# niess/turtle

Hardware: AMD Instinct MI355X
Metric: ray-steps/sec (whole node) through 3601^2 SRTM tile (higher is better)
Workload: dtype f64

## Files before the change

### turtle_amd/csrc/device.hip

```cpp
#include <hip/hip_runtime.h>
#include <hipcub/device/device_radix_sort.hpp>

#include <cfloat>
#include <cstdio>
#include <cstdlib>
#include <cstring>
#include <type_traits>

#include "device_ctx.h"
#include "internal.h"
#include "trace_room.h"

using namespace turtle_amd_device;

namespace {


__device__ __forceinline__ int lane_rank(ull mask)
{
        return __builtin_amdgcn_mbcnt_hi((unsigned)(mask >> 32), __builtin_amdgcn_mbcnt_lo((unsigned)mask, 0));
}

struct RayQueue {
        long next = 0, end = 0;
// ... 2157 lines not shown
        }
        block_tally(stats, my_rays, my_steps, my_samples, my_capped);
}

__global__ void k_traverse_gen(long n, int first, const double * __restrict__ alt,
    const double * __restrict__ step, int * __restrict__ live_index, int * __restrict__ medium,
    int * __restrict__ index, double * __restrict__ length, int * __restrict__ n_steps,
    int * __restrict__ n_cross, double ceiling, int max_steps, ull * __restrict__ counters)
{
        ull my_rays = 0, my_steps = 0, my_capped = 0, my_live = 0;
        for (long r = blockIdx.x * (long)blockDim.x + threadIdx.x; r < n;
             r += (long)gridDim.x * blockDim.x) {
                const int m1 = live_index[2 * r];
                int count = 0;
                if (first) {
                        n_steps[r] = 0, n_cross[r] = 0;
                } else {
                        const int m0 = medium[r];
                        if (m0 < 0) continue;
                        if (length != nullptr) length[(long)m0 * n + r] += step[r];
                        count = n_steps[r] + 1;
                        n_steps[r] = count;
                        n_cross[r] += (m1 != m0) ? 1 : 0;
                        my_steps++;
                }
                index[2 * r] = m1, index[2 * r + 1] = live_index[2 * r + 1];
                const bool low = (m1 >= 0) && (alt[r] < ceiling);
                if (!low || (count >= max_steps)) {
                        medium[r] = -1, live_index[2 * r] = -1;
                        my_rays++;
                        my_capped += low ? 1 : 0;
                } else {
                        medium[r] = m1;
                        my_live++;
                }
        }
        block_tally(counters, my_rays, my_steps, my_capped, my_live);
}

__global__ void k_crossings_gen(long n, const double * __restrict__ pos, const double * __restrict__ step,
    const int * __restrict__ live_index, const int * __restrict__ medium, const int * __restrict__ n_cross,
    double * __restrict__ total, tamd_crossings rec)
{
        for (long r = blockIdx.x * (long)blockDim.x + threadIdx.x; r < n;
             r += (long)gridDim.x * blockDim.x) {
                const int m0 = medium[r];
                if (m0 < 0) continue;
                const double tot = total[r] + step[r];
                total[r] = tot;
                const int m1 = live_index[2 * r];
                if ((m1 != m0) && (n_cross[r] < rec.capacity)) {
                        const long c = (long)n_cross[r] * n + r;
                        if (rec.point != nullptr)
                                rec.point[3 * c] = pos[3 * r], rec.point[3 * c + 1] = pos[3 * r + 1],
                                rec.point[3 * c + 2] = pos[3 * r + 2];
                        if (rec.distance != nullptr) rec.distance[c] = tot;
                        if (rec.media != nullptr) rec.media[2 * c] = m0, rec.media[2 * c + 1] = m1;
                }
        }
}

__global__ void k_philox(long n, ull seed, ull stream, long first, unsigned * __restrict__ out)
{
        for (long r = blockIdx.x * (long)blockDim.x + threadIdx.x; r < n;
             r += (long)gridDim.x * blockDim.x) {
                const ull id = (ull)(first + r);
                unsigned c[4] = { (unsigned)id, (unsigned)(id >> 32), (unsigned)stream,
                        (unsigned)(stream >> 32) };
                philox4x32_10(c, (unsigned)seed, (unsigned)(seed >> 32));
                for (int i = 0; i < 4; i++) out[4 * r + i] = c[i];
        }
}

__global__ void k_isotropic(long n, ull seed, ull stream, long first, double * __restrict__ dir)
{
        for (long r = blockIdx.x * (long)blockDim.x + threadIdx.x; r < n;
             r += (long)gridDim.x * blockDim.x) {
                double x, y, z;
                d_isotropic((ull)(first + r), stream, seed, x, y, z);
                dir[3 * r] = x, dir[3 * r + 1] = y, dir[3 * r + 2] = z;
        }
}

__global__ void __launch_bounds__(256) k_tally(long n, const int * __restrict__ index,
    const double * __restrict__ length, int n_media, ull * __restrict__ hits,
    int n_bins, double scale, ull * __restrict__ histogram)
{
        extern __shared__ unsigned int lds[];
        unsigned int * h_hits = lds;
        unsigned int * h_bins = lds + (n_media + 1);
        const int total = n_media + 1 + n_bins + 1;
        for (int i = threadIdx.x; i < total; i += blockDim.x) lds[i] = 0;
        __syncthreads();
        for (long r = blockIdx.x * (long)blockDim.x + threadIdx.x; r < n;
             r += (long)gridDim.x * blockDim.x) {
                const int m = index[2 * r];
                if ((m >= -1) && (m < n_media)) atomicAdd(&h_hits[m + 1], 1u);
                const double t = length[r] * scale;
                int b = n_bins;
                if ((t >= 0.) && (t < (double)n_bins)) b = (int)t;
                atomicAdd(&h_bins[b], 1u);
        }
        __syncthreads();
        for (int i = threadIdx.x; i < total; i += blockDim.x) {
                const unsigned int c = lds[i];
                if (c == 0) continue;
                if (i <= n_media)
                        atomicAdd(&hits[i], (ull)c);
                else
                        atomicAdd(&histogram[i - (n_media + 1)], (ull)c);
        }
}

enum { RS_STACK = 0, RS_MAP = 1 };

__device__ __forceinline__ void page_fault_block(const Paging & pg, const TileFault & f, int item)
{
        const bool fault = f.centre >= 0;
        const ull mask = __ballot(fault);
        if (mask == 0) return;
        const int lane = (int)(threadIdx.x & 63);
        const int leader = __builtin_ctzll(mask);
        ull base = 0;
        if (lane == leader) {
                base = atomicAdd(pg.n_faulted, 1ull);
                pg.faulted[base] = item;
        }
        base = __shfl(base, leader, 64);
        const bool first = (pg.first_id >= 0) ? (item == pg.first_id) : (base == 0);
        if (fault) {
                for (int b = 0; b < 9; b++) {
                        if (!((f.mask >> b) & 1)) continue;
                        const int t = f.centre + (b / 3 - 1) * f.stride + (b % 3 - 1);
                        if (b != 4) atomicAdd(&pg.wanted[(size_t)t * TAMD_DEMAND_STRIDE], 1u);
                        if (first) atomicOr(&pg.wanted_first[t >> 5], 1u << (t & 31));
                }
        }
        const bool centre = fault && (((f.mask >> 4) & 1) != 0);
        ull left = __ballot(centre);
        while (left != 0) {
                const int lead = __builtin_ctzll(left);
                const int t0 = __shfl(f.centre, lead, 64);
                const ull same = __ballot(centre && (f.centre == t0));
                if (lane == lead) atomicAdd(&pg.wanted[(size_t)t0 * TAMD_DEMAND_STRIDE], 1u);
                left &= ~same;
        }
}

template <int SRC, int TPROJ >
__global__ void __launch_bounds__(256) k_resample(tamd_view v, const tamd_grid * __restrict__ grids,
    double z0, double dz, int is_signed, int flags, long n_blocks, uint16_t * __restrict__ out, Paging pg,
    ull * __restrict__ counters)
{
        const tamd_grid & t = grids[0];
        const int lane = (int)(threadIdx.x & 63);
        const long waves = (long)gridDim.x * (blockDim.x >> 6);
        const long n_items = (pg.n_in != nullptr) ? (long)*pg.n_in : n_blocks;
        const double top = z0 + 65535 * dz;
        ull n_outside = 0, n_bad = 0, n_clamped = 0;
        for (long i = blockIdx.x * (long)(blockDim.x >> 6) + (threadIdx.x >> 6); i < n_items; i += waves) {
                const long blk = (pg.ids != nullptr) ? (long)pg.ids[i] : i;
                const int ix = (int)(blk % t.nbx) * TAMD_BLOCK + (lane & 7);
                const int iy = (int)(blk / t.nbx) * TAMD_BLOCK + (lane >> 3);
                TileFault f = { -1, 0, 0 };
                bool keep = true;
                int outside = 0, bad = 0, clamped = 0;
                uint16_t code = 0;
                if ((ix < t.nx) && (iy < t.ny)) {
                        const double x = t.x0 + ix * t.dx;
                        const double y = t.y0 + iy * t.dy;
                        double latitude, longitude;
                        if (TPROJ >= 0)
                                d_unproject_body<TPROJ>(t.proj, x, y, latitude, longitude);
                        else
                                latitude = y, longitude = x;
                        double z = 0.;
                        int in;
                        if (SRC == RS_STACK) {
                                in = d_stack_elevation<false>(v, v.stacks[0], latitude, longitude, z, f);
                                if (in >= 0) f.centre = -1;
                        } else {
                                const tamd_grid & s = grids[1];
                                double u, w;
                                if (flags & TAMD_RESAMPLE_IDENTITY)
                                        u = x, w = y;
                                else if (s.proj.type >= 0)
                                        d_project_body(s.proj, latitude, longitude, u, w);
                                else
                                        u = longitude, w = latitude;
                                in = d_grid_elevation<false>(s, u, w, z) ? 1 : 0;
                        }
                        if (in == 0) {
                                outside = 1;
                        } else if (in > 0) {
// ... 57 lines not shown
                        if (is_signed)
                                code = (uint16_t)(int)z;
                        else
                                code = (dz > 0.) ? (uint16_t)(unsigned)round((z - z0) / dz) : 0;
                }
                codes[k] = code;
        }
        block_tally(counters, n_bad, n_clamped, n_inconsistent, 0);
}

__global__ void __launch_bounds__(256) k_fill_store(uint16_t * __restrict__ nodes, int nbx, int ix0, int iy0,
    int nx, int ny, int nwx, long n_blocks, int blank, const uint16_t * __restrict__ codes)
{
        const int lane = (int)(threadIdx.x & 63);
        const long waves = (long)gridDim.x * (blockDim.x >> 6);
        for (long i = blockIdx.x * (long)(blockDim.x >> 6) + (threadIdx.x >> 6); i < n_blocks; i += waves) {
                const int bx = (ix0 >> 3) + (int)(i % nwx), by = (iy0 >> 3) + (int)(i / nwx);
                const int ix = bx * TAMD_BLOCK + (lane & 7) - ix0, iy = by * TAMD_BLOCK + (lane >> 3) - iy0;
                const size_t k = ((size_t)by * nbx + bx) * 64 + lane;
                uint16_t code = 0;
                if ((ix >= 0) && (ix < nx) && (iy >= 0) && (iy < ny))
                        code = codes[(long)iy * nx + ix];
                else if (!blank)
                        code = GLOBAL_NODES(nodes)[k];
                nodes[k] = code;
        }
}

__global__ void __launch_bounds__(256) k_nodes(const uint16_t * __restrict__ nodes, int nbx, int ix0, int iy0,
    int nx, long n, double z0, double dz, int is_signed, double * __restrict__ out, long ld)
{
        for (long k = blockIdx.x * (long)blockDim.x + threadIdx.x; k < n; k += (long)gridDim.x * blockDim.x) {
                const long j = k / nx;
                const int i = (int)(k - j * nx);
                const uint16_t code = GLOBAL_NODES(nodes)[d_node_index(nbx, ix0 + i, iy0 + (int)j)];
                out[j * ld + i] = is_signed ? (double)(int16_t)code : z0 + code * dz;
        }
}

}


#define g_stream (g_ctx.stream)
#define g_cus (g_ctx.cus)
#define g_math_strict (g_ctx.math_strict)

#ifdef TRACE_POOL_STATS
extern "C" int tamd_dev_pool_stats(unsigned long long * out, int reset)
{
        HIP_TRY(hipMemcpyFromSymbol(out, HIP_SYMBOL(g_pool_stats), sizeof(g_pool_stats)));
        if (reset) {
                static unsigned long long zero[32];
                HIP_TRY(hipMemcpyToSymbol(HIP_SYMBOL(g_pool_stats), zero, sizeof(zero)));
        }
        return 0;
}
#endif

static int grid_for(long n, int block)
{
        long blocks = (n + block - 1) / block;
        const long cap = (long)(g_cus > 0 ? g_cus : 256) * 8;
        if (blocks > cap) blocks = cap;
        if (blocks < 1) blocks = 1;
        return (int)blocks;
}

template <class... P, class... A>
static int launch_blocks(const char * name, void (*kernel)(P...), unsigned blocks, size_t lds_bytes,
    const A &... args)
{
        hipLaunchKernelGGL(kernel, dim3(blocks), dim3(256), lds_bytes, g_stream, args...);
        LAUNCH_CHECK(name);
        return 0;
}
template <class... P, class... A>
static int launch_items(const char * name, void (*kernel)(P...), long n, size_t lds_bytes, const A &... args)
{
        if (tamd_dev_init()) return 1;
        if (n <= 0) return 0;
        return launch_blocks(name, kernel, grid_for(n, 256), lds_bytes, args...);
}

template <int FIRST, int... REST, class F>
static int with_constant(int value, F && f)
{
        if constexpr (sizeof...(REST) > 0)
                if (value != FIRST) return with_constant<REST...>(value, f);
        return f(std::integral_constant<int, FIRST>());
}
template <class F>
static int with_mode(int mode, F && f)
{
        return with_constant<TAMD_MODE_ONE_MAP, TAMD_MODE_ONE_STACK, TAMD_MODE_GENERIC>(mode, f);
}

typedef std::integral_constant<int, 0> Strict;
typedef std::integral_constant<int, 1> Fast;
template <class F>
static int with_math(bool strict, F && f)
{
        return with_constant<Strict::value, Fast::value>(strict ? Strict::value : Fast::value, f);
}

extern "C" int tamd_k_ecef_from_geodetic(long n, const double * lat,
    const double * lon, const double * elev, double * ecef)
{
        return launch_items("k_ecef_from_geodetic", k_ecef_from_geodetic, n, 0, n, lat, lon, elev, ecef);
}

extern "C" int tamd_k_ecef_to_geodetic(
    long n, const double * ecef, double * lat, double * lon, double * alt)
{
        return with_math(g_math_strict, [&](auto fast) {
                return launch_items("k_ecef_to_geodetic", k_ecef_to_geodetic<decltype(fast)::value>, n, 0, n,
                    ecef, lat, lon, alt);
        });
}

extern "C" int tamd_k_ecef_from_horizontal(long n, const double * lat,
    const double * lon, const double * az, const double * el, double * dir)
{
        return launch_items("k_ecef_from_horizontal", k_ecef_from_horizontal, n, 0, n, lat, lon, az, el, dir);
}

extern "C" int tamd_k_ecef_to_horizontal(long n, const double * lat,
    const double * lon, const double * dir, double * az, double * el)
{
        return launch_items("k_ecef_to_horizontal", k_ecef_to_horizontal, n, 0, n, lat, lon, dir, az, el);
}

extern "C" int tamd_k_elevation(struct tamd_view view, long n, const double * a,
    const double * b, double * z, int * inside, struct tamd_paging pg)
{
        return launch_items("k_elevation", k_elevation, n, 0, view, n, a, b, z, inside, pg);
}

extern "C" int tamd_k_project(struct tamd_proj proj, int inverse, long n, const double * a,
    const double * b, double * c, double * d)
{
        return launch_items("k_project", k_project, n, 0, proj, inverse, n, a, b, c, d);
}

extern "C" int tamd_k_gradient(struct tamd_view view, long n, const double * a,
    const double * b, double * ga, double * gb, int * inside, struct tamd_paging pg)
{
        return launch_items("k_gradient", k_gradient, n, 0, view, n, a, b, ga, gb, inside, pg);
}

extern "C" int tamd_k_position(struct tamd_view view, long n, const double * lat,
    const double * lon, const double * height, int layer, double * pos,
    int * data_index, struct tamd_paging pg)
{
        return launch_items("k_position", k_position, n, 0, view, n, lat, lon, height, layer, pos,
            data_index, pg);
}

extern "C" int tamd_k_normal(struct tamd_view view, long n, const double * pos, const int * layer,
    double * normal, int * data_index, struct tamd_paging pg)
{
        return with_mode(view.mode, [&](auto mode) {
                return launch_items("k_normal", k_normal<decltype(mode)::value>, n, 0, view, n, pos, layer,
                    normal, data_index, pg);
        });
}

// ... 124 lines not shown
        }
        if constexpr (FAST && MODEL && (MODE != TAMD_MODE_GENERIC))
                if (cross && (ph.pool > 0)) return launch_trace_<MODE, FAST, MODEL, false, true, true>(TRACE_ARGS);
        if (cross) return launch_trace_<MODE, FAST, MODEL, false, true>(TRACE_ARGS);
        if constexpr (!MODEL) return launch_trace_<MODE, FAST, MODEL, false, false>(TRACE_ARGS);
        return 1;
#undef TRACE_ARGS
}

struct TraceRays {
        double * pos;
        const double * dir;
        int * index;
        double * length;
        int * n_steps;
};

template <int MODE, bool FAST>
static int launch_cross(struct tamd_view view, long n, const TraceRays & rays, CrossList cross, Paging pg,
    ull * stats, RayOut out = { nullptr, nullptr, nullptr, nullptr, nullptr }, CrossTail front = { nullptr })
{
        constexpr bool CAN_PAGE = (MODE != TAMD_MODE_ONE_MAP);
        const bool paged = CAN_PAGE && (pg.faulted != nullptr);
        const auto kernel = paged ? k_cross<MODE, FAST, CAN_PAGE> : k_cross<MODE, FAST, false>;
        return launch_blocks("k_cross", kernel, persistent_blocks(kernel, n), 0, view, rays.pos, rays.dir, rays.index,
            rays.length, rays.n_steps, cross, pg, stats, out, front, n);
}


struct Knob {
        const char * name;
        long fallback;
        bool read = false;
        long value = 0;
        long get()
        {
                if (!read) {
                        const char * env = getenv(name);
                        value = ((env != nullptr) && (*env != 0)) ? atol(env) : fallback;
                        read = true;
                }
                return value;
        }
};

static int park_threshold(int mode)
{
        static Knob knob = { "TURTLE_AMD_PARK", -1 };
        const int value = (int)knob.get();
        if (value >= 0) return value;
        return (mode == TAMD_MODE_GENERIC) ? 512 : 32;
}
static int creep_lanes(long n)
{
        static Knob knob = { "TURTLE_AMD_CREEP_LANES", -1 };
        const int value = (int)knob.get();
        if (value >= 0) return value;
        return (n >= 2000000) ? 4 * kCreepLanes : kCreepLanes;
}
static int dense_go(void)
{
        static Knob knob = { "TURTLE_AMD_DENSE_GO", 24 };
        return (int)knob.get();
}
static int sort_long_if(void)
{
        static Knob knob = { "TURTLE_AMD_SORT_LONG", 120 };
        return (int)knob.get();
}
static int pool_on(int mode, long n)
{
        static Knob knob = { "TURTLE_AMD_POOL", -1 };
        const int value = (int)knob.get();
        if (value >= 0) return value;
        return (mode == TAMD_MODE_ONE_MAP) && (n >= 6000000);
}
static int sort_hand_over(long n)
{
        static Knob knob = { "TURTLE_AMD_SORT_KEY", -1 };
        const long value = knob.get();
        if (value == 0) return 0;
        if (value == 1) return 1;
        return n <= ((value > 1) ? value : 4000000L);
}
static int spatial_order(int mode, long n)
{
        static Knob knob = { "TURTLE_AMD_SPATIAL", -1 };
        const long value = knob.get();
        if ((mode == TAMD_MODE_GENERIC) || (value == 0)) return 0;
        if (value == 1) return 1;
        return n >= ((value > 1) ? value : 3000000L);
}
static int cross_tail_on(long n)
{
        static Knob knob = { "TURTLE_AMD_CROSS_TAIL", -1 };
        const long value = knob.get();
        if (value >= 0) return value != 0;
        return (g_ctx.in_flight <= 1) && (n <= 3000000L);
}
constexpr int kDrainLanes = 64;
static bool first_pass_flat(int park, bool again, const Paging & pg)
{
        static Knob knob = { "TURTLE_AMD_FIRST_PASS", -1 };
        if (knob.get() == 0) return false;
        return !again && (pg.faulted == nullptr) && (park > 0) && (park <= 64);
}
static int first_pass_waves(bool ordered)
{
        static Knob knob = { "TURTLE_AMD_FIRST_WAVES", -1 };
        if (knob.get() > 0) return (knob.get() <= 3) ? 3 : 8;
        return ordered ? 8 : 3;
}
template <int MODE>
static int launch_first(struct tamd_view view, long n, double * pos, const double * dir, int max_steps,
    int * index, double * length, int * n_steps, int flags, const FirstPass & fp, const RayOut & out, ull * stats)
{
        static Knob grid = { "TURTLE_AMD_FIRST_GRID", 1 };
        if (tamd_dev_init()) return 1;
        const unsigned blocks = (grid.get() == 0) ? (unsigned)grid_for(n, 256) : (unsigned)((n + 255) / 256);
        return with_constant<3, 8>(first_pass_waves(out.order_of != nullptr), [&](auto waves) {
                return launch_blocks("k_first", k_first<MODE, decltype(waves)::value>, blocks, 0, view, n, pos, dir,
                    max_steps, index, length, n_steps, flags, fp, out, stats);
        });
}


static ull * counter_of(ull * queue, enum tamd_trace_counter c) { return queue + (int)c * kQ; }
static_assert(((int)TAMD_TRACE_TAIL_N_DRY - (int)TAMD_TRACE_QUEUE_B) * kQ == kQTail,
    "CrossTail.n_dry is kQTail words behind the lined pass's queue");
static_assert(((int)TAMD_TRACE_TAIL_L1_NEXT == (int)TAMD_TRACE_TAIL_N_DRY + 1) &&
        ((int)TAMD_TRACE_TAIL_L2_COUNT == (int)TAMD_TRACE_TAIL_N_DRY + 2),
    "CrossTail.l1_next and .l2_count follow n_dry, kQ words apart");

template <class KEY>
struct RoomSort {
        static_assert(sizeof(KEY) <= sizeof(int), "a key buffer holds an int a ray (trace_room.h)");
        hipcub::DoubleBuffer<KEY> keys;
        hipcub::DoubleBuffer<int> ids;
        void * temp;
        size_t temp_bytes;
        int n, bits;
        RoomSort(char * room, const tamd_trace_room & at, long n_, int bits_)
            : keys(TAMD_ROOM_AT(KEY, room, at.keys), TAMD_ROOM_AT(KEY, room, at.keys_alt)),
              ids(TAMD_ROOM_AT(int, room, at.parked), TAMD_ROOM_AT(int, room, at.ids_alt)),
              temp(room + at.sort_temp), temp_bytes(0), n((int)n_), bits(bits_)
        {
        }
        bool fits()
        {
                return (hipcub::DeviceRadixSort::SortPairs(nullptr, temp_bytes, keys, ids, n, 0, bits, g_stream) ==
                           hipSuccess) &&
                    (temp_bytes <= TAMD_TRACE_SORT_TEMP);
        }
        int run()
        {
                if (hipcub::DeviceRadixSort::SortPairs(temp, temp_bytes, keys, ids, n, 0, bits, g_stream) != hipSuccess)
                        return fail("hipcub::DeviceRadixSort", hipGetLastError());
                return 0;
        }
};

template <int MODE>
static int order_rays(struct tamd_view view, long n, char * room, const tamd_trace_room & at, TraceRays & rays,
    PhaseIO & a, PhaseIO & b, RayOut & out)
{
        RoomSort<SPATIAL_KEY_T> sort(room, at, n, SPATIAL_BITS);
        if (!sort.fits()) return 0;
        hipLaunchKernelGGL(k_ray_cells<MODE>, dim3(grid_for(n, 256)), dim3(256), 0, g_stream, view, n, rays.pos,
            sort.keys.Current(), sort.ids.Current());
        LAUNCH_CHECK("k_ray_cells");
        if (sort.run()) return 1;
        int * const kept = TAMD_ROOM_AT(int, room, at.order);
        HIP_TRY(hipMemcpyAsync(kept, sort.ids.Current(), (size_t)n * sizeof(int), hipMemcpyDeviceToDevice, g_stream));
        out.order_of = kept, out.pos = rays.pos, out.index = rays.index, out.length = rays.length;
        out.n_steps = rays.n_steps;
        a.out = out, b.out = out;
        a.pos_in = rays.pos, a.dir_in = rays.dir, a.index_in = rays.index;
        a.dir_copy = TAMD_ROOM_AT(double, room, at.dir_s);
        rays.pos = TAMD_ROOM_AT(double, room, at.pos_s), rays.dir = a.dir_copy;
        rays.index = TAMD_ROOM_AT(int, room, at.index_s), rays.length = TAMD_ROOM_AT(double, room, at.length_s);
        rays.n_steps = TAMD_ROOM_AT(int, room, at.n_steps_s);
        return 0;
}

static int hand_over_plan(RoomSort<unsigned char> & sort, long n, bool again, ull * queue, double * ds_mark,
    PhaseIO & a, PhaseIO & b, bool & sorting)
{
        const int long_if = sort_long_if();
        sorting = false;
        if (again || (long_if <= 0)) return 0;
        a.n_parked_back = counter_of(queue, TAMD_TRACE_N_PARKED_BACK);
        a.ds_mark = ds_mark, a.mark_at = a.park_after / 2, a.long_if = (float)long_if;
        b.n_dev_back = a.n_parked_back;
        sorting = sort_hand_over(n) && sort.fits();
        if (!sorting) return 0;
        a.sort_key = sort.keys.Current();
        HIP_TRY(hipMemsetAsync(a.sort_key, 0xFE, (size_t)n, g_stream));
        return 0;
}
static int hand_over_sort(RoomSort<unsigned char> & sort, PhaseIO & b)
{
        if (sort.run()) return 1;
        b.ids = sort.ids.Current();
        return 0;
}

template <int MODE, int FAST>
static int launch_plain(struct tamd_view view, long n, bool again, const TraceRays & rays, int max_steps, int flags,
    const PhaseIO & ph, ull * stats, ull * queue)
{
        return launch_trace<MODE, FAST != 0, false>(view, n, again, rays.pos, rays.dir, max_steps, rays.index,
            rays.length, rays.n_steps, flags, ph, stats, counter_of(queue, TAMD_TRACE_QUEUE_A));
}

template <int MODE>
static int launch_phase_a(struct tamd_view view, long n, bool again, const TraceRays & rays, int max_steps, int flags,
    const PhaseIO & a, const RayOut & out, ull * stats, ull * queue)
{
        if constexpr (MODE != TAMD_MODE_GENERIC) {
                if (first_pass_flat(a.park_after, again, a.pg)) {
                        const FirstPass fp = { a.park_after, a.mark_at, a.long_if, a.parked, a.n_parked,
                                a.n_parked_back, a.sort_key, a.cross, a.pos_in, a.dir_in, a.index_in, a.dir_copy };
                        return launch_first<MODE>(view, n, rays.pos, rays.dir, max_steps, rays.index, rays.length,
                            rays.n_steps, flags, fp, out, stats);
                }
        }
        return launch_plain<MODE, Fast::value>(view, n, again, rays, max_steps, flags, a, stats, queue);
}

template <int MODE>
static int launch_lined(struct tamd_view view, long n, const TraceRays & rays, int max_steps, int flags,
    const PhaseIO & b, const CrossTail & tail, ull * stats, ull * queue)
{
        const int tail_flag = (tail.words != nullptr) ? TRACE_CROSS_TAIL : 0;
        return launch_trace<MODE, true, true>(view, n, true, rays.pos, rays.dir, max_steps, rays.index, rays.length,
            rays.n_steps, flags | TRACE_CARRY_MEDIUM | tail_flag, b, stats, counter_of(queue, TAMD_TRACE_QUEUE_B));
}

template <int MODE>
static int run_trace(struct tamd_view view, long n, TraceRays rays, int max_steps, int flags, char * room,
    Paging pg, ull * stats, ull * queue)
{
        const bool again = (pg.ids != nullptr);
        if (again) flags |= TRACE_CARRY_MEDIUM;
        const bool strict = g_math_strict || !view.fast_ok;
        const bool listed = (room != nullptr) && (rays.length != nullptr) && (rays.n_steps != nullptr);
        tamd_trace_room at;
        tamd_trace_room_layout(&at, n);
        CrossList cross = { nullptr, nullptr, nullptr, nullptr };
        if (listed) {
                cross.ray = TAMD_ROOM_AT(int, room, at.cross_ray), cross.ds = TAMD_ROOM_AT(double, room, at.cross_ds);
                cross.count = counter_of(queue, TAMD_TRACE_N_CROSS);
                cross.other = TAMD_ROOM_AT(int, room, at.cross_other);
        }
        PhaseIO shared = {};
        shared.pg = pg, shared.chunk = kChunk, shared.creep_lanes = creep_lanes(n), shared.dense_go = dense_go();
        shared.cross = cross;
        PhaseIO one = shared;
        one.ids = pg.ids, one.n_dev = pg.n_in, one.accumulate = again ? 2 : 0;
        if (!listed)
                return with_math(strict, [&](auto fast) {
                        return launch_plain<MODE, decltype(fast)::value>(view, n, again, rays, max_steps, flags, one,
                            stats, queue);
                });
        if (strict) {
                if (launch_plain<MODE, Strict::value>(view, n, again, rays, max_steps, flags, one, stats, queue)) return 1;
                return launch_cross<MODE, false>(view, n, rays, cross, pg, stats);
        }
        const int park = park_threshold(MODE);
        if ((park <= 0) || (max_steps <= park)) {
                if (launch_plain<MODE, Fast::value>(view, n, again, rays, max_steps, flags, one, stats, queue)) return 1;
                return launch_cross<MODE, true>(view, n, rays, cross, pg, stats);
        }
        PhaseIO a = one, b = shared;
        a.parked = TAMD_ROOM_AT(int, room, at.parked), a.n_parked = counter_of(queue, TAMD_TRACE_N_PARKED);
        a.park_after = park, a.drain_lanes = kDrainLanes;
        b.ids = a.parked, b.n_dev = a.n_parked, b.accumulate = 1, b.line_after = park;
        b.pool = pool_on(MODE, n);
        CrossTail tail = { nullptr };
        if ((MODE != TAMD_MODE_GENERIC) && (pg.faulted == nullptr) && cross_tail_on(n))
                tail.words = counter_of(queue, TAMD_TRACE_TAIL_N_DRY);
        RayOut out = { nullptr, nullptr, nullptr, nullptr, nullptr };
        if constexpr (MODE != TAMD_MODE_GENERIC) {
                if (!again && (pg.faulted == nullptr) && spatial_order(MODE, n))
                        if (order_rays<MODE>(view, n, room, at, rays, a, b, out)) return 1;
        }
        RoomSort<unsigned char> hand_over(room, at, n, 8);
        bool sorting = false;
        if (hand_over_plan(hand_over, n, again, queue, TAMD_ROOM_AT(double, room, at.ds_mark), a, b, sorting)) return 1;
        if (launch_phase_a<MODE>(view, n, again, rays, max_steps, flags, a, out, stats, queue)) return 1;
        if (sorting && hand_over_sort(hand_over, b)) return 1;
        if (launch_lined<MODE>(view, n, rays, max_steps, flags, b, tail, stats, queue)) return 1;
        return launch_cross<MODE, true>(view, n, rays, cross, pg, stats, out, tail);
}

extern "C" int tamd_k_trace(struct tamd_view view, long n, double * pos,
    const double * dir, int max_steps, int * index, double * length, int * n_steps,
    int flags, void * room, struct tamd_paging pg, unsigned long long * stats,
    unsigned long long * queue)
{
        if (tamd_dev_init()) return 1;
        if ((pos == nullptr) || (dir == nullptr) || (index == nullptr) || (stats == nullptr) ||
            (queue == nullptr) ||
            ((pg.faulted != nullptr) &&
                ((pg.tentative == nullptr) || (length == nullptr) || (n_steps == nullptr) ||
                    (pg.n_faulted == nullptr) || (pg.wanted == nullptr) || (pg.wanted_first == nullptr)))) {
                snprintf(g_error, sizeof(g_error), "tamd_k_trace: a required array is missing");
                return 1;
        }
        if (pg.ids == nullptr) HIP_TRY(hipMemsetAsync(stats, 0, 4 * sizeof(ull), g_stream));
        HIP_TRY(hipMemsetAsync(queue, 0, TAMD_TRACE_COUNTERS * sizeof(ull), g_stream));
        if (n <= 0) return 0;
        const int carry = (flags & TURTLE_AMD_TRACE_RESUME) ? TRACE_CARRY_MEDIUM : 0;
        const TraceRays rays = { pos, dir, index, length, n_steps };
        return with_mode(view.mode, [&](auto mode) {
                return run_trace<decltype(mode)::value>(view, n, rays, max_steps, carry, (char *)room, pg, stats, queue);
        });
}

extern "C" int tamd_k_step_dir(struct tamd_view view, long n, double * pos,
    const double * dir, double * lat, double * lon, double * alt, double * elev,
    double * step, int * index, int flags, int * cross_ray, double * cross_ds,
    struct tamd_paging pg, unsigned long long * stats, unsigned long long * queue)
{
        if (tamd_dev_init()) return 1;
        if (pg.ids == nullptr) HIP_TRY(hipMemsetAsync(stats, 0, 4 * sizeof(ull), g_stream));
        HIP_TRY(hipMemsetAsync(queue, 0, 3 * sizeof(ull), g_stream));
        if (n <= 0) return 0;
        const CrossList cross = { cross_ray, (cross_ray != nullptr) ? cross_ds : nullptr, queue + 2, nullptr };
        const StepWalk no_walk = { 0, 0, 0, 0, nullptr, nullptr };
        return run_step(view, n, pos, dir, lat, lon, alt, elev, step, index, flags, cross, pg,
            stats, no_walk);
}

extern "C" int tamd_k_step_walk(struct tamd_view view, long n, double * pos, double * alt,
    double * elev, int * index, unsigned long long seed, unsigned long long stream, long first,
    double * length, int * steps, int * cross_ray, double * cross_ds, struct tamd_paging pg,
    unsigned long long * stats, unsigned long long * queue)
{
        if (tamd_dev_init()) return 1;
        HIP_TRY(hipMemsetAsync(queue, 0, 3 * sizeof(ull), g_stream));
        if (n <= 0) return 0;
        const CrossList cross = { cross_ray, cross_ds, queue + 2, nullptr };
        const StepWalk walk = { 1, seed, stream, first, length, steps };
        return run_step(view, n, pos, nullptr, nullptr, nullptr, alt, elev, nullptr, index,
            TURTLE_AMD_STEP_RESUME, cross, pg, stats, walk);
}

extern "C" int tamd_k_walk(struct tamd_view view, long n, double * pos, double * alt, double * elev,
    int * index, unsigned long long seed, long first, int first_step, int n_steps, double * length,
    int * steps, unsigned long long * stats, unsigned long long * queue)
{
        if (tamd_dev_init()) return 1;
        HIP_TRY(hipMemsetAsync(queue, 0, sizeof(ull), g_stream));
        if (n <= 0) return 0;
        const WalkIO io = { seed, first, first_step, n_steps };
        const bool strict = g_math_strict || !view.fast_ok;
        return with_mode(view.mode, [&](auto mode) {
                return with_math(strict, [&](auto fast) {
                        const auto kernel = k_walk<decltype(mode)::value, decltype(fast)::value>;
                        return launch_blocks("k_walk", kernel, persistent_blocks(kernel, n), 0, view, n, pos, alt,
                            elev, index, length, steps, io, stats, queue);
                });
        });
}

template <int MODE, bool REC>
static int launch_traverse(const tamd_view & view, long n, double * pos, int * index, const TraverseIO & io,
    ull * stats, ull * queue, bool strict, typename CrossingsArg<REC>::type rec)
{
        return with_math(strict, [&](auto fast) {
                const auto kernel = k_traverse<MODE, decltype(fast)::value, REC>;
                return launch_blocks("k_traverse", kernel, persistent_blocks(kernel, n), 0, view, n, pos, index, io,
                    stats, queue, rec);
        });
}

extern "C" int tamd_k_traverse(struct tamd_view view, long n, double * pos, const double * dir,
    double ceiling, int max_steps, int * index, double * length, int * n_steps, int * n_cross,
    const struct tamd_crossings * rec, unsigned long long * stats, unsigned long long * queue)
{
        if (tamd_dev_init()) return 1;
        HIP_TRY(hipMemsetAsync(stats, 0, 4 * sizeof(ull), g_stream));
        HIP_TRY(hipMemsetAsync(queue, 0, sizeof(ull), g_stream));
        if (n <= 0) return 0;
        const TraverseIO io = { dir, length, n_steps, n_cross, ceiling, max_steps };
        const bool strict = g_math_strict || !view.fast_ok;
        return with_mode(view.mode, [&](auto mode) {
                constexpr int MODE = decltype(mode)::value;
                if (rec != nullptr)
                        return launch_traverse<MODE, true>(view, n, pos, index, io, stats, queue, strict, *rec);
                return launch_traverse<MODE, false>(view, n, pos, index, io, stats, queue, strict, NoCrossings());
        });
}

extern "C" int tamd_k_step_live(struct tamd_view view, long n, double * pos, const double * dir,
    double * alt, double * elev, double * step, int * index, int * cross_ray, double * cross_ds,
    struct tamd_paging pg, unsigned long long * stats, unsigned long long * queue)
{
        if (tamd_dev_init()) return 1;
        HIP_TRY(hipMemsetAsync(queue, 0, 3 * sizeof(ull), g_stream));
        if (n <= 0) return 0;
        const CrossList cross = { cross_ray, (cross_ray != nullptr) ? cross_ds : nullptr, queue + 2, nullptr };
        const StepWalk no_walk = { 0, 0, 0, 0, nullptr, nullptr };
        return run_step(view, n, pos, dir, nullptr, nullptr, alt, elev, step, index,
            TURTLE_AMD_STEP_RESUME | TAMD_STEP_LIVE, cross, pg, stats, no_walk);
}

extern "C" int tamd_k_traverse_gen(long n, int first, const double * alt, const double * step,
    int * live_index, int * medium, int * index, double * length, int * n_steps, int * n_cross,
    double ceiling, int max_steps, unsigned long long * counters)
{
        return launch_items("k_traverse_gen", k_traverse_gen, n, 0, n, first, alt, step, live_index, medium,
            index, length, n_steps, n_cross, ceiling, max_steps, counters);
}

extern "C" int tamd_k_crossings_gen(long n, const double * pos, const double * step, const int * live_index,
    const int * medium, const int * n_cross, double * total, struct tamd_crossings rec)
{
        return launch_items("k_crossings_gen", k_crossings_gen, n, 0, n, pos, step, live_index, medium, n_cross,
            total, rec);
}

extern "C" int tamd_k_philox(long n, unsigned long long seed, unsigned long long stream,
    long first, unsigned * out)
{
        return launch_items("k_philox", k_philox, n, 0, n, seed, stream, first, out);
}

extern "C" int tamd_k_isotropic(long n, unsigned long long seed, unsigned long long stream,
    long first, double * dir)
{
        return launch_items("k_isotropic", k_isotropic, n, 0, n, seed, stream, first, dir);
}

extern "C" int tamd_k_tally(long n, const int * index, const double * length,
    int n_media, unsigned long long * hits, int n_bins, double length_max,
    unsigned long long * histogram)
{
        if (tamd_dev_init()) return 1;
        if (n <= 0) return 0;
        const size_t lds = (size_t)(n_media + 1 + n_bins + 1) * sizeof(unsigned int);
        if (lds > 64 * 1024) {
                snprintf(g_error, sizeof(g_error), "too many tally bins (%d)", n_bins);
                return 1;
        }
        const double scale = (double)n_bins / length_max;
        return launch_blocks("k_tally", k_tally, grid_for(n, 256), lds, n, index, length, n_media, hits, n_bins, scale,
            histogram);
}

extern "C" int tamd_k_resample(struct tamd_view view, const struct tamd_grid * grids, int from_map,
    double z0, double dz, int is_signed, int flags, long n_blocks, uint16_t * out,
    struct tamd_paging pg, unsigned long long * counters)
{
        if (tamd_dev_init()) return 1;
        if (n_blocks <= 0) return 0;
        struct tamd_grid target;
        if (tamd_dev_d2h(&target, grids, sizeof(target))) return 1;
        const unsigned blocks = grid_for(n_blocks * 64, 256);
        return with_constant<RS_MAP, RS_STACK>(from_map ? RS_MAP : RS_STACK, [&](auto source) {
                return with_constant<TAMD_PROJ_LAMBERT, TAMD_PROJ_UTM, TAMD_PROJ_NONE>(target.proj.type, [&](auto type) {
                        return launch_blocks("k_resample", k_resample<decltype(source)::value, decltype(type)::value>,
                            blocks, 0, view, grids, z0, dz, is_signed, flags, n_blocks, out, pg, counters);
                });
        });
}

extern "C" int tamd_k_unblock(const uint16_t * blocked, int nx, int ny, int nbx, uint16_t * rows)
{
        return launch_items("k_unblock", k_unblock, (long)nx * ny, 0, blocked, nx, ny, nbx, rows);
}

extern "C" int tamd_k_fill_encode(const double * elevation, long ld, int nx, int ny, double z0, double dz,
    int is_signed, int flags, uint16_t * codes, unsigned long long * counters)
{
        const long n = (long)nx * ny;
        return launch_items("k_fill_encode", k_fill_encode, n, 0, elevation, ld, nx, n, z0, dz, is_signed, flags,
            codes, counters);
}

extern "C" int tamd_k_fill_store(uint16_t * nodes, int nbx, int ix0, int iy0, int nx, int ny, int blank,
    const uint16_t * codes)
{
        const int nwx = ((ix0 + nx - 1) >> 3) - (ix0 >> 3) + 1, nwy = ((iy0 + ny - 1) >> 3) - (iy0 >> 3) + 1;
        const long n_blocks = (long)nwx * nwy;
        return launch_items("k_fill_store", k_fill_store, n_blocks * 64, 0, nodes, nbx, ix0, iy0, nx, ny, nwx,
            n_blocks, blank, codes);
}

extern "C" int tamd_k_nodes(const uint16_t * nodes, int nbx, int ix0, int iy0, int nx, int ny, double z0,
    double dz, int is_signed, double * elevation, long ld)
{
        const long n = (long)nx * ny;
        return launch_items("k_nodes", k_nodes, n, 0, nodes, nbx, ix0, iy0, nx, n, z0, dz, is_signed, elevation, ld);
}
```

### turtle_amd/csrc/internal.h

```cpp
#ifndef TURTLE_AMD_INTERNAL_H
#define TURTLE_AMD_INTERNAL_H

#include <stddef.h>
#include <stdint.h>

#include "turtle_amd.h"
#include "turtle_amd_device.h"

#ifdef __cplusplus
extern "C" {
#endif



const char * tamd_dev_error(void);
int tamd_dev_init(void);
void tamd_dev_release(void);
int tamd_dev_sync_device(int device);
void tamd_dev_free_on(int device, void * ptr);
int tamd_dev_block(int which, void ** ptr, size_t bytes, int * grown);
#define TAMD_MAX_DEVICES 16
int tamd_dev_count(void);
int tamd_dev_select(int device);
int tamd_dev_current(void);
int tamd_dev_cus(void);
int tamd_dev_stream_set(void * stream);
int tamd_dev_sync(void);
void tamd_dev_math_set(int strict);
int tamd_dev_math_get(void);
void tamd_dev_in_flight_set(int batches);
int tamd_dev_in_flight_get(void);

int tamd_dev_malloc(void ** ptr, size_t bytes);
void tamd_dev_free(void * ptr);
int tamd_dev_h2d(void * dst, const void * src, size_t bytes);
int tamd_dev_d2h(void * dst, const void * src, size_t bytes);
int tamd_dev_zero(void * dst, size_t bytes);
int tamd_dev_pinned(void ** ptr, size_t bytes);
int tamd_dev_copy_async(void * dst, const void * src, size_t bytes, int to_device);
int tamd_dev_host_alloc(void ** ptr, size_t bytes);
void tamd_dev_host_free(void * ptr);

void tamd_scratch_reset(void);
int tamd_scratch_get(void ** ptr, size_t bytes);

#define TAMD_DEMAND_STRIDE 32
struct tamd_paging {
        const int * ids;
        const unsigned long long * n_in;
        int * faulted;
        unsigned long long * n_faulted;
        unsigned * wanted;
        unsigned * wanted_first;
        double * tentative;
        int first_id;
};

int tamd_k_ecef_from_geodetic(long n, const double * lat, const double * lon,
    const double * elev, double * ecef);
int tamd_k_ecef_to_geodetic(long n, const double * ecef, double * lat,
    double * lon, double * alt);
int tamd_k_ecef_from_horizontal(long n, const double * lat, const double * lon,
    const double * az, const double * el, double * dir);
int tamd_k_ecef_to_horizontal(long n, const double * lat, const double * lon,
    const double * dir, double * az, double * el);
int tamd_k_elevation(struct tamd_view view, long n, const double * a,
    const double * b, double * z, int * inside, struct tamd_paging pg);
int tamd_k_gradient(struct tamd_view view, long n, const double * a,
    const double * b, double * ga, double * gb, int * inside, struct tamd_paging pg);
int tamd_k_position(struct tamd_view view, long n, const double * lat,
    const double * lon, const double * height, int layer, double * pos,
    int * data_index, struct tamd_paging pg);
int tamd_k_normal(struct tamd_view view, long n, const double * pos, const int * layer,
    double * normal, int * data_index, struct tamd_paging pg);
int tamd_k_horizon(struct tamd_view view, int n_items, int n_azimuths, int n_distances,
    const double * pos, const double * azimuth, const double * distance, int layer, double * elevation,
    int * sample, double * range);
int tamd_k_viewshed(struct tamd_view view, int n_items, int n_azimuths, int n_distances,
    const double * pos, const double * azimuth, const double * distance, int layer, double target_height,
    signed char * visible, double * sine, double * horizon, int * n_visible);
int tamd_k_clearance(struct tamd_view view, int n_items, int n_targets, int paired, int n_fractions,
    const double * observer, const double * target, const double * fraction, int layer, double * clearance,
    int * sample, int * n_data);
int tamd_k_step(struct tamd_view view, long n, double * pos,
    const double * dir, double * lat, double * lon, double * alt,
    double * elev, double * step, int * index, int flags, struct tamd_paging pg);
enum tamd_trace_counter {
        TAMD_TRACE_QUEUE_A = 0,
        TAMD_TRACE_QUEUE_B,
        TAMD_TRACE_N_PARKED,
        TAMD_TRACE_N_CROSS,
        TAMD_TRACE_N_PARKED_BACK,
        TAMD_TRACE_TAIL_N_DRY,
        TAMD_TRACE_TAIL_L1_NEXT,
        TAMD_TRACE_TAIL_L2_COUNT,
        TAMD_TRACE_N_COUNTERS
};
#define TAMD_TRACE_COUNTER_STRIDE 16
#define TAMD_TRACE_COUNTERS (TAMD_TRACE_N_COUNTERS * TAMD_TRACE_COUNTER_STRIDE)
#define TAMD_STATS_QUEUE 4
#define TAMD_STATS_STEPS (TAMD_STATS_QUEUE + TAMD_TRACE_COUNTERS)
#define TAMD_STATS_WORDS (TAMD_STATS_STEPS + 4)
int tamd_k_trace(struct tamd_view view, long n, double * pos,
    const double * dir, int max_steps, int * index, double * length,
    int * n_steps, int flags, void * room, struct tamd_paging pg,
    unsigned long long * stats, unsigned long long * queue);
#define TAMD_STEP_COMPACT 0x200
int tamd_k_step_dir(struct tamd_view view, long n, double * pos,
    const double * dir, double * lat, double * lon, double * alt,
    double * elev, double * step, int * index, int flags, int * cross_ray,
    double * cross_ds, struct tamd_paging pg, unsigned long long * stats,
    unsigned long long * queue);
int tamd_k_step_walk(struct tamd_view view, long n, double * pos, double * alt,
    double * elev, int * index, unsigned long long seed, unsigned long long stream, long first,
    double * length, int * steps, int * cross_ray, double * cross_ds, struct tamd_paging pg,
    unsigned long long * stats, unsigned long long * queue);
int tamd_k_walk(struct tamd_view view, long n, double * pos, double * alt, double * elev,
    int * index, unsigned long long seed, long first, int first_step, int n_steps, double * length,
    int * steps, unsigned long long * stats, unsigned long long * queue);
#define TAMD_STEP_LIVE 0x400
struct tamd_crossings {
        double * point;
        double * distance;
        int * media;
        int capacity;
};
int tamd_k_traverse(struct tamd_view view, long n, double * pos, const double * dir,
    double ceiling, int max_steps, int * index, double * length, int * n_steps, int * n_cross,
    const struct tamd_crossings * rec, unsigned long long * stats, unsigned long long * queue);
int tamd_k_step_live(struct tamd_view view, long n, double * pos, const double * dir,
    double * alt, double * elev, double * step, int * index, int * cross_ray, double * cross_ds,
    struct tamd_paging pg, unsigned long long * stats, unsigned long long * queue);
int tamd_k_traverse_gen(long n, int first, const double * alt, const double * step, int * live_index,
    int * medium, int * index, double * length, int * n_steps, int * n_cross, double ceiling,
    int max_steps, unsigned long long * counters);
int tamd_k_crossings_gen(long n, const double * pos, const double * step, const int * live_index,
    const int * medium, const int * n_cross, double * total, struct tamd_crossings rec);
int tamd_k_philox(long n, unsigned long long seed, unsigned long long stream,
    long first, unsigned * out);
int tamd_k_isotropic(long n, unsigned long long seed, unsigned long long stream,
    long first, double * dir);
int tamd_k_project(struct tamd_proj proj, int inverse, long n, const double * a,
    const double * b, double * c, double * d);
int tamd_k_tally(long n, const int * index, const double * length,
    int n_media, unsigned long long * hits, int n_bins, double length_max,
    unsigned long long * histogram);
#define TAMD_RESAMPLE_IDENTITY 0x100
int tamd_k_resample(struct tamd_view view, const struct tamd_grid * grids, int from_map,
    double z0, double dz, int is_signed, int flags, long n_blocks, uint16_t * out,
    struct tamd_paging pg, unsigned long long * counters);
int tamd_k_unblock(const uint16_t * blocked, int nx, int ny, int nbx, uint16_t * rows);
int tamd_k_fill_encode(const double * elevation, long ld, int nx, int ny, double z0, double dz,
    int is_signed, int flags, uint16_t * codes, unsigned long long * counters);
int tamd_k_fill_store(uint16_t * nodes, int nbx, int ix0, int iy0, int nx, int ny, int blank,
    const uint16_t * codes);
int tamd_k_nodes(const uint16_t * nodes, int nbx, int ix0, int iy0, int nx, int ny, double z0,
    double dz, int is_signed, double * elevation, long ld);

#ifdef __cplusplus
}
#endif
#endif
```

Before: 72.33 billion.

## Replace hipcub hand-over sort with custom byte-key counting order; widen tally kernel

Replaces the hipcub radix sort used to reorder rays at the phase hand-over with two custom kernels that count byte keys per block and place ids by prefix sum with atomic cursors. This removes the key memset and the multi-pass radix sort, at the cost of a non-stable order within buckets. The tally kernel moves to 1024-thread blocks with replicated LDS histograms and ballot-based medium counting to cut LDS atomic contention. Separate stats and queue memsets are also merged into one where the buffers are contiguous.

```diff
diff --git a/turtle_amd/csrc/device.hip b/turtle_amd/csrc/device.hip
--- a/turtle_amd/csrc/device.hip
+++ b/turtle_amd/csrc/device.hip
@@ -2263,34 +2263,135 @@
         }
 }
 
-__global__ void __launch_bounds__(256) k_tally(long n, const int * __restrict__ index,
+constexpr int kTallyThreads = 1024;
+constexpr int kTallyBallotMedia = 7;
+
+__global__ void __launch_bounds__(kTallyThreads) k_tally(long n, const int * __restrict__ index,
     const double * __restrict__ length, int n_media, ull * __restrict__ hits,
-    int n_bins, double scale, ull * __restrict__ histogram)
+    int n_bins, double scale, ull * __restrict__ histogram, int copies)
 {
         extern __shared__ unsigned int lds[];
         unsigned int * h_hits = lds;
         unsigned int * h_bins = lds + (n_media + 1);
-        const int total = n_media + 1 + n_bins + 1;
+        const int total = n_media + 1 + copies * (n_bins + 1);
         for (int i = threadIdx.x; i < total; i += blockDim.x) lds[i] = 0;
         __syncthreads();
-        for (long r = blockIdx.x * (long)blockDim.x + threadIdx.x; r < n;
-             r += (long)gridDim.x * blockDim.x) {
-                const int m = index[2 * r];
-                if ((m >= -1) && (m < n_media)) atomicAdd(&h_hits[m + 1], 1u);
-                const double t = length[r] * scale;
-                int b = n_bins;
-                if ((t >= 0.) && (t < (double)n_bins)) b = (int)t;
-                atomicAdd(&h_bins[b], 1u);
-        }
+        const int lane = threadIdx.x & 63;
+        unsigned int * my_bins = h_bins + (size_t)((threadIdx.x >> 6) % copies) * (n_bins + 1);
+        const bool by_ballot = (n_media <= kTallyBallotMedia);
+        unsigned int my_hits = 0;
+        for (long first = blockIdx.x * (long)blockDim.x + (threadIdx.x - lane); first < n;
+             first += (long)gridDim.x * blockDim.x) {
+                const long r = first + lane;
+                const bool live = (r < n);
+                int m = -2;
+                if (live) {
+                        m = index[2 * r];
+                        const double t = length[r] * scale;
+                        int b = n_bins;
+                        if ((t >= 0.) && (t < (double)n_bins)) b = (int)t;
+                        atomicAdd(&my_bins[b], 1u);
+                }
+                if (by_ballot) {
+                        for (int j = 0; j <= n_media; j++) {
+                                const unsigned int c = (unsigned int)__popcll(__ballot(m + 1 == j));
+                                if (lane == j) my_hits += c;
+                        }
+                } else if ((m >= -1) && (m < n_media))
+                        atomicAdd(&h_hits[m + 1], 1u);
+        }
+        if (by_ballot && (lane <= n_media) && (my_hits != 0)) atomicAdd(&h_hits[lane], my_hits);
         __syncthreads();
-        for (int i = threadIdx.x; i < total; i += blockDim.x) {
-                const unsigned int c = lds[i];
-                if (c == 0) continue;
-                if (i <= n_media)
-                        atomicAdd(&hits[i], (ull)c);
-                else
-                        atomicAdd(&histogram[i - (n_media + 1)], (ull)c);
-        }
+        for (int i = threadIdx.x; i < n_media + 1 + n_bins + 1; i += blockDim.x) {
+                if (i <= n_media) {
+                        if (h_hits[i] != 0) atomicAdd(&hits[i], (ull)h_hits[i]);
+                        continue;
+                }
+                const int b = i - (n_media + 1);
+                unsigned int c = 0;
+                for (int k = 0; k < copies; k++) c += h_bins[(size_t)k * (n_bins + 1) + b];
+                if (c != 0) atomicAdd(&histogram[b], (ull)c);
+        }
+}
+
+constexpr int kOrderThreads = 1024;
+constexpr int kOrderBlocks = 256;
+constexpr int kOrderBins = TAMD_ORDER_BINS;
+
+struct OrderSpan {
+        long n_front, n_back;
+        long lo, hi;
+};
+__device__ __forceinline__ OrderSpan order_span(long n, const ull * __restrict__ n_front,
+    const ull * __restrict__ n_back)
+{
+        OrderSpan s;
+        s.n_front = min((long)min(*n_front, (ull)n), n);
+        s.n_back = (n_back != nullptr) ? (long)min(*n_back, (ull)(n - s.n_front)) : 0;
+        const long chunk = ((s.n_front + gridDim.x - 1) / gridDim.x + 15) & ~15L;
+        s.lo = min(s.n_front, blockIdx.x * chunk);
+        s.hi = min(s.n_front, s.lo + chunk);
+        return s;
+}
+template <class F>
+__device__ __forceinline__ void order_each(const unsigned char * __restrict__ keys, long lo, long hi, F && f)
+{
+        for (long i = lo + 4L * threadIdx.x; i < hi; i += 4L * blockDim.x) {
+                if (i + 4 <= hi) {
+                        const unsigned int four = *(const unsigned int *)(keys + i);
+                        for (int k = 0; k < 4; k++) f(i + k, (int)((four >> (8 * k)) & 255u));
+                } else
+                        for (long j = i; j < hi; j++) f(j, (int)keys[j]);
+        }
+}
+
+__global__ void __launch_bounds__(kOrderThreads) k_order_count(long n, const unsigned char * __restrict__ keys,
+    const ull * __restrict__ n_front, const ull * __restrict__ n_back, unsigned int * __restrict__ counts)
+{
+        __shared__ unsigned int mine[kOrderBins];
+        const OrderSpan s = order_span(n, n_front, n_back);
+        if (s.lo >= s.hi) return;
+        if (threadIdx.x < kOrderBins) mine[threadIdx.x] = 0;
+        __syncthreads();
+        order_each(keys, s.lo, s.hi, [&](long, int key) { atomicAdd(&mine[key], 1u); });
+        __syncthreads();
+        if ((threadIdx.x < kOrderBins) && (mine[threadIdx.x] != 0)) atomicAdd(&counts[threadIdx.x], mine[threadIdx.x]);
+}
+
+__global__ void __launch_bounds__(kOrderThreads) k_order_place(long n, const unsigned char * __restrict__ keys,
+    const int * __restrict__ ids, const ull * __restrict__ n_front, const ull * __restrict__ n_back,
+    const unsigned int * __restrict__ counts, unsigned int * __restrict__ cursors, int * __restrict__ out)
+{
+        __shared__ unsigned int mine[kOrderBins];
+        __shared__ unsigned int wave_sum[kOrderBins / 64];
+        const OrderSpan s = order_span(n, n_front, n_back);
+        for (long i = blockIdx.x * (long)blockDim.x + threadIdx.x; i < s.n_back; i += (long)gridDim.x * blockDim.x)
+                out[n - s.n_back + i] = ids[n - s.n_back + i];
+        if (s.lo >= s.hi) return;
+        const int t = threadIdx.x, lane = t & 63;
+        if (t < kOrderBins) mine[t] = 0;
+        __syncthreads();
+        order_each(keys, s.lo, s.hi, [&](long, int key) { atomicAdd(&mine[key], 1u); });
+        const unsigned int count = (t < kOrderBins) ? counts[t] : 0;
+        unsigned int upto = count;
+        for (int d = 1; d < 64; d <<= 1) {
+                const unsigned int below = __shfl_up(upto, d, 64);
+                if (lane >= d) upto += below;
+        }
+        if ((t < kOrderBins) && (lane == 63)) wave_sum[t >> 6] = upto;
+        __syncthreads();
+        if (t < kOrderBins) {
+                unsigned int begin = upto - count;
+                for (int w = 0; w < (t >> 6); w++) begin += wave_sum[w];
+                const unsigned int held = mine[t];
+                const unsigned int taken = (held != 0) ? atomicAdd(&cursors[t], held) : 0;
+                mine[t] = begin + taken;
+        }
+        __syncthreads();
+        order_each(keys, s.lo, s.hi, [&](long place, int key) {
+                const unsigned int to = atomicAdd(&mine[key], 1u);
+                if ((long)to < s.n_front) out[to] = ids[place];
+        });
 }
 
 enum { RS_STACK = 0, RS_MAP = 1 };
@@ -2514,6 +2615,17 @@
         return launch_blocks(name, kernel, grid_for(n, 256), lds_bytes, args...);
 }
 
+static int zero_words(ull * stats, int n_stats, ull * queue, int n_queue)
+{
+        if ((n_stats > 0) && (queue == stats + TAMD_STATS_QUEUE) && (n_stats <= TAMD_STATS_QUEUE)) {
+                HIP_TRY(hipMemsetAsync(stats, 0, (size_t)(TAMD_STATS_QUEUE + n_queue) * sizeof(ull), g_stream));
+                return 0;
+        }
+        if (n_stats > 0) HIP_TRY(hipMemsetAsync(stats, 0, (size_t)n_stats * sizeof(ull), g_stream));
+        HIP_TRY(hipMemsetAsync(queue, 0, (size_t)n_queue * sizeof(ull), g_stream));
+        return 0;
+}
+
 template <int FIRST, int... REST, class F>
 static int with_constant(int value, F && f)
 {
@@ -2804,6 +2916,11 @@
         if (value == 0) return 0;
         if (value == 1) return 1;
         return n <= ((value > 1) ? value : 4000000L);
+}
+static int sort_own(void)
+{
+        static Knob knob = { "TURTLE_AMD_SORT_OWN", 1 };
+        return knob.get() != 0;
 }
 static int spatial_order(int mode, long n)
 {
@@ -2914,14 +3031,34 @@
         a.n_parked_back = counter_of(queue, TAMD_TRACE_N_PARKED_BACK);
         a.ds_mark = ds_mark, a.mark_at = a.park_after / 2, a.long_if = (float)long_if;
         b.n_dev_back = a.n_parked_back;
-        sorting = sort_hand_over(n) && sort.fits();
+        sorting = sort_hand_over(n) && (sort_own() || sort.fits());
         if (!sorting) return 0;
         a.sort_key = sort.keys.Current();
-        HIP_TRY(hipMemsetAsync(a.sort_key, 0xFE, (size_t)n, g_stream));
+        if (!sort_own()) HIP_TRY(hipMemsetAsync(a.sort_key, 0xFE, (size_t)n, g_stream));
         return 0;
 }
-static int hand_over_sort(RoomSort<unsigned char> & sort, PhaseIO & b)
-{
+static int launch_order(long n, const int * ids, const unsigned char * keys, const ull * n_front, const ull * n_back,
+    unsigned int * words, int * out)
+{
+        const long wanted = (n + 4 * kOrderThreads - 1) / (4 * kOrderThreads);
+        const unsigned blocks = (unsigned)((wanted < 1) ? 1 : (wanted > kOrderBlocks) ? kOrderBlocks : wanted);
+        hipLaunchKernelGGL(k_order_count, dim3(blocks), dim3(kOrderThreads), 0, g_stream, n, keys, n_front, n_back,
+            words);
+        LAUNCH_CHECK("k_order_count");
+        hipLaunchKernelGGL(k_order_place, dim3(blocks), dim3(kOrderThreads), 0, g_stream, n, keys, ids, n_front,
+            n_back, words, words + kOrderBins, out);
+        LAUNCH_CHECK("k_order_place");
+        return 0;
+}
+static int hand_over_sort(RoomSort<unsigned char> & sort, long n, const PhaseIO & a, ull * queue, PhaseIO & b)
+{
+        if (sort_own()) {
+                if (launch_order(n, sort.ids.Current(), sort.keys.Current(), a.n_parked, a.n_parked_back,
+                        (unsigned int *)(queue + TAMD_TRACE_COUNTERS), sort.ids.Alternate()))
+                        return 1;
+                b.ids = sort.ids.Alternate();
+                return 0;
+        }
         if (sort.run()) return 1;
         b.ids = sort.ids.Current();
         return 0;
@@ -3011,7 +3148,7 @@
         bool sorting = false;
         if (hand_over_plan(hand_over, n, again, queue, TAMD_ROOM_AT(double, room, at.ds_mark), a, b, sorting)) return 1;
         if (launch_phase_a<MODE>(view, n, again, rays, max_steps, flags, a, out, stats, queue)) return 1;
-        if (sorting && hand_over_sort(hand_over, b)) return 1;
+        if (sorting && hand_over_sort(hand_over, n, a, queue, b)) return 1;
         if (launch_lined<MODE>(view, n, rays, max_steps, flags, b, tail, stats, queue)) return 1;
         return launch_cross<MODE, true>(view, n, rays, cross, pg, stats, out, tail);
 }
@@ -3030,8 +3167,7 @@
                 snprintf(g_error, sizeof(g_error), "tamd_k_trace: a required array is missing");
                 return 1;
         }
-        if (pg.ids == nullptr) HIP_TRY(hipMemsetAsync(stats, 0, 4 * sizeof(ull), g_stream));
-        HIP_TRY(hipMemsetAsync(queue, 0, TAMD_TRACE_COUNTERS * sizeof(ull), g_stream));
+        if (zero_words(stats, (pg.ids == nullptr) ? 4 : 0, queue, TAMD_TRACE_QUEUE_WORDS)) return 1;
         if (n <= 0) return 0;
         const int carry = (flags & TURTLE_AMD_TRACE_RESUME) ? TRACE_CARRY_MEDIUM : 0;
         const TraceRays rays = { pos, dir, index, length, n_steps };
@@ -3046,8 +3182,7 @@
     struct tamd_paging pg, unsigned long long * stats, unsigned long long * queue)
 {
         if (tamd_dev_init()) return 1;
-        if (pg.ids == nullptr) HIP_TRY(hipMemsetAsync(stats, 0, 4 * sizeof(ull), g_stream));
-        HIP_TRY(hipMemsetAsync(queue, 0, 3 * sizeof(ull), g_stream));
+        if (zero_words(stats, (pg.ids == nullptr) ? 4 : 0, queue, 3)) return 1;
         if (n <= 0) return 0;
         const CrossList cross = { cross_ray, (cross_ray != nullptr) ? cross_ds : nullptr, queue + 2, nullptr };
         const StepWalk no_walk = { 0, 0, 0, 0, nullptr, nullptr };
@@ -3103,8 +3238,7 @@
     const struct tamd_crossings * rec, unsigned long long * stats, unsigned long long * queue)
 {
         if (tamd_dev_init()) return 1;
-        HIP_TRY(hipMemsetAsync(stats, 0, 4 * sizeof(ull), g_stream));
-        HIP_TRY(hipMemsetAsync(queue, 0, sizeof(ull), g_stream));
+        if (zero_words(stats, 4, queue, 1)) return 1;
         if (n <= 0) return 0;
         const TraverseIO io = { dir, length, n_steps, n_cross, ceiling, max_steps };
         const bool strict = g_math_strict || !view.fast_ok;
@@ -3168,8 +3302,31 @@
                 return 1;
         }
         const double scale = (double)n_bins / length_max;
-        return launch_blocks("k_tally", k_tally, grid_for(n, 256), lds, n, index, length, n_media, hits, n_bins, scale,
-            histogram);
+        static Knob block = { "TURTLE_AMD_TALLY_THREADS", kTallyThreads };
+        const int threads = ((block.get() == 256) || (block.get() == 512)) ? (int)block.get() : kTallyThreads;
+        const long cus = (g_cus > 0) ? g_cus : 256;
+        long blocks = (n + threads - 1) / threads;
+        if (blocks > cus) blocks = cus;
+        const size_t one = (size_t)(n_bins + 1) * sizeof(unsigned int);
+        size_t copies = (64 * 1024 - (size_t)(n_media + 1) * sizeof(unsigned int)) / one;
+        if (copies > (size_t)threads / 64) copies = (size_t)threads / 64;
+        hipLaunchKernelGGL(k_tally, dim3((unsigned)blocks), dim3(threads),
+            (size_t)(n_media + 1) * sizeof(unsigned int) + copies * one, g_stream, n, index, length, n_media, hits,
+            n_bins, scale, histogram, (int)copies);
+        LAUNCH_CHECK("k_tally");
+        return 0;
+}
+
+extern "C" int tamd_k_hand_over_order(long n, const int * ids, const unsigned char * keys,
+    const unsigned long long * n_front, const unsigned long long * n_back, unsigned int * words, int * out)
+{
+        if (tamd_dev_init()) return 1;
+        if (n <= 0) return 0;
+        if ((ids == nullptr) || (keys == nullptr) || (n_front == nullptr) || (words == nullptr) || (out == nullptr)) {
+                snprintf(g_error, sizeof(g_error), "tamd_k_hand_over_order: a required array is missing");
+                return 1;
+        }
+        return launch_order(n, ids, keys, n_front, n_back, words, out);
 }
 
 extern "C" int tamd_k_resample(struct tamd_view view, const struct tamd_grid * grids, int from_map,
diff --git a/turtle_amd/csrc/internal.h b/turtle_amd/csrc/internal.h
--- a/turtle_amd/csrc/internal.h
+++ b/turtle_amd/csrc/internal.h
@@ -98,13 +98,26 @@
 };
 #define TAMD_TRACE_COUNTER_STRIDE 16
 #define TAMD_TRACE_COUNTERS (TAMD_TRACE_N_COUNTERS * TAMD_TRACE_COUNTER_STRIDE)
+#define TAMD_ORDER_BINS 256
+#define TAMD_TRACE_ORDER_WORDS (2 * TAMD_ORDER_BINS * 4 / 8)
+#define TAMD_TRACE_QUEUE_WORDS (TAMD_TRACE_COUNTERS + TAMD_TRACE_ORDER_WORDS)
 #define TAMD_STATS_QUEUE 4
-#define TAMD_STATS_STEPS (TAMD_STATS_QUEUE + TAMD_TRACE_COUNTERS)
+#define TAMD_STATS_ORDER (TAMD_STATS_QUEUE + TAMD_TRACE_COUNTERS)
+#define TAMD_STATS_STEPS (TAMD_STATS_QUEUE + TAMD_TRACE_QUEUE_WORDS)
 #define TAMD_STATS_WORDS (TAMD_STATS_STEPS + 4)
+#if defined(__cplusplus)
+static_assert(TAMD_STATS_ORDER + TAMD_TRACE_ORDER_WORDS == TAMD_STATS_STEPS,
+    "stats, the trace's counters and the ordering's words are one contiguous run of d_stats");
+#else
+_Static_assert(TAMD_STATS_ORDER + TAMD_TRACE_ORDER_WORDS == TAMD_STATS_STEPS,
+    "stats, the trace's counters and the ordering's words are one contiguous run of d_stats");
+#endif
 int tamd_k_trace(struct tamd_view view, long n, double * pos,
     const double * dir, int max_steps, int * index, double * length,
     int * n_steps, int flags, void * room, struct tamd_paging pg,
     unsigned long long * stats, unsigned long long * queue);
+int tamd_k_hand_over_order(long n, const int * ids, const unsigned char * keys,
+    const unsigned long long * n_front, const unsigned long long * n_back, unsigned int * words, int * out);
 #define TAMD_STEP_COMPACT 0x200
 int tamd_k_step_dir(struct tamd_view view, long n, double * pos,
     const double * dir, double * lat, double * lon, double * alt,
```

Measured after the change: 73.92 billion (median of 6 runs). 2.2% higher.
